# stanford-iprl-lab/nerf_shared

Hardware: AMD Instinct MI355X
Metric: rays_per_sec (higher is better)
Workload: dtype bf16; 1 GPU; lego_halfres_400x400_64c+128f_viewdirs_8x256_chunk4096; entry=Renderer.render(c2w=pose, retraw=False), chunk=4096, N_samples=64, N_importance=128, weights=random-init seeds 0/10, parallelism=single GPU

## Files before the change

nerf_shared_amd/csrc/capi.hip:

```cpp
#include <hip/hip_runtime.h>

#include <cmath>

#include <cstdio>
#include <cstring>
#include <mutex>
#include <utility>
#include <new>
#include <string>
#include <vector>

#include "kernels.h"
#include "program.h"

using namespace na;

namespace {
thread_local std::string g_err;

std::string lds_msg(const char *what, size_t bytes) {
    return std::string(what) + ": the per-ray scratch needs " + std::to_string(bytes) + " bytes of LDS per workgroup, the CU has " +
           std::to_string(LDS_LIMIT_BYTES) + " (fewer samples per ray)";
}

// ... 539 lines not shown
    if (Ni > 0 && !io->u && !io->t_lin_imp) return fail(NERF_AMD_EINVAL, "need u or t_lin_imp for sample_pdf");
    const nerf_amd_model *fm = fine ? fine : coarse;
    const int och = coarse->prog.out_ch;
    if (Ni > 0 && fm->prog.out_ch != och) return fail(NERF_AMD_EINVAL, "coarse and fine models disagree on output channels");
    if (och < 4) return fail(NERF_AMD_EINVAL, "field must output at least 4 channels");
    const bool has_vd = io->ray_ch > 8;
    if ((coarse->prog.arch.use_viewdirs != 0) != has_vd || (fm->prog.arch.use_viewdirs != 0) != has_vd)
        return fail(NERF_AMD_EINVAL, "ray batch width does not match the models' use_viewdirs");
    if (io->workspace_bytes < nerf_amd_render_rays_workspace(cfg, R, och) || !io->workspace)
        return fail(NERF_AMD_EINVAL, "workspace too small");
    p->cfg = cfg; p->coarse = coarse; p->fm = fm; p->io = io; p->R = R;
    p->Nc = Nc; p->Ni = Ni; p->Nf = Nf; p->och = och; p->has_vd = has_vd;

    char *w = static_cast<char *>(io->workspace);
    auto take = [&](size_t bytes) { float *q = reinterpret_cast<float *>(w); w += align_up(bytes); return q; };
    p->z_c = take(R * Nc * sizeof(float));
    p->raw_c = take(R * Nc * och * sizeof(float));
    p->w_c = take(R * Nc * sizeof(float));
    p->z_f = p->raw_f = nullptr;
    if (Ni > 0) {
        p->z_f = take(R * (size_t)Nf * sizeof(float));
        p->raw_f = take(R * (size_t)Nf * och * sizeof(float));
        if (io->z_vals) p->z_f = io->z_vals;
        if (io->raw) p->raw_f = io->raw;
    } else {
        if (io->z_vals) p->z_c = io->z_vals;
        if (io->raw) p->raw_c = io->raw;
        if (io->weights) p->w_c = io->weights;
    }
    return NERF_AMD_OK;
}

int stage_z(ChunkPlan &p, hipStream_t s) {
    const nerf_amd_render_io *io = p.io;
    int rc = 0;
    if (io->z_coarse) {
        if (p.Ni == 0 && io->z_vals)
            rc = hipMemcpyAsync(io->z_vals, io->z_coarse, p.R * p.Nc * sizeof(float), hipMemcpyDeviceToDevice, s) == hipSuccess
                     ? 0 : NERF_AMD_EHIP;
        else
            p.z_c = const_cast<float *>(io->z_coarse);
    } else {
        rc = launch_coarse_z(io->rays, io->ray_ch, io->t_vals, p.cfg->perturb ? io->t_rand : nullptr, p.R, p.Nc,
                             p.cfg->lindisp, p.cfg->perturb, p.z_c, s);
    }
    return rc ? fail(rc, "coarse_z launch failed") : NERF_AMD_OK;
}

int stage_field(const ChunkPlan &p, bool fine_pass, hipStream_t s) {
    MlpArgs a;
    std::memset(&a, 0, sizeof(a));
    a.rays = p.io->rays; a.ray_stride = p.io->ray_ch;
    a.viewdirs = p.has_vd ? p.io->rays + 8 : nullptr; a.vd_stride = p.io->ray_ch;
    if (!fine_pass) {
        a.z_vals = p.z_c; a.P = p.R * p.Nc; a.S = p.Nc; a.out = p.raw_c;
        return run_field(p.coarse, a, p.cfg->precision, s);
    }
    a.z_vals = p.z_f; a.P = p.R * (int64_t)p.Nf; a.S = p.Nf; a.out = p.raw_f;
    return run_field(p.fm, a, p.cfg->precision, s);
}

CompositeJob final_job(const ChunkPlan &p) {
    const nerf_amd_render_io *io = p.io;
    CompositeJob j;
    std::memset(&j, 0, sizeof(j));
    const bool two_pass = p.Ni > 0;
    j.raw = two_pass ? p.raw_f : p.raw_c; j.raw_ch = p.och; j.z = two_pass ? p.z_f : p.z_c;
    j.rays_d = io->rays + 3; j.rays_d_stride = io->ray_ch;
    j.noise = p.cfg->use_noise ? (two_pass ? io->noise1 : io->noise0) : nullptr;
    j.R = p.R; j.S = two_pass ? p.Nf : p.Nc; j.white_bkgd = p.cfg->white_bkgd;
    j.rgb = io->rgb_map; j.disp = io->disp_map; j.acc = io->acc_map; j.weights = two_pass ? io->weights : p.w_c;
    return j;
}

int stage_final(const ChunkPlan &p, hipStream_t s) {
    const CompositeJob j = final_job(p);
    int rc = launch_composite(j.raw, j.raw_ch, j.z, j.rays_d, j.rays_d_stride, j.noise, j.R, j.S, j.white_bkgd, j.rgb, j.disp,
                              j.acc, j.weights, nullptr, s);
    return rc ? fail(rc, "composite launch failed") : NERF_AMD_OK;
}

int stage_mid(const ChunkPlan &p, const ChunkPlan *prev, hipStream_t s) {
    const nerf_amd_render_io *io = p.io;
    CompositeJob cj;
    std::memset(&cj, 0, sizeof(cj));
    cj.raw = p.raw_c; cj.raw_ch = p.och; cj.z = p.z_c; cj.rays_d = io->rays + 3; cj.rays_d_stride = io->ray_ch;
    cj.noise = p.cfg->use_noise ? io->noise0 : nullptr; cj.R = p.R; cj.S = p.Nc; cj.white_bkgd = p.cfg->white_bkgd;
    cj.rgb = io->rgb0; cj.disp = io->disp0; cj.acc = io->acc0; cj.weights = nullptr;
    ResampleJob rj;
    std::memset(&rj, 0, sizeof(rj));
    rj.u = io->u; rj.t_lin = io->t_lin_imp; rj.Ni = p.Ni; rj.z_fine = p.z_f; rj.z_std = io->z_std;
    CompositeJob fj;
    if (prev) fj = final_job(*prev);
    int rc = launch_mid_stage(cj, rj, prev ? &fj : nullptr, s);
    if (rc == NERF_AMD_EINVAL && resample_lds_bytes(p.Nc, p.Ni, true) > LDS_LIMIT_BYTES)
        return fail(rc, lds_msg("render_rays (compositing + resampling)", resample_lds_bytes(p.Nc, p.Ni, true)));
    return rc ? fail(rc, "composite/resample launch failed") : NERF_AMD_OK;
}
}

extern "C" {

int nerf_amd_render_rays(const nerf_amd_render_cfg *cfg, const nerf_amd_model *coarse, const nerf_amd_model *fine,
                         const nerf_amd_render_io *io, int64_t R, void *stream) {
    if (R == 0 && cfg && coarse && io) return NERF_AMD_OK;
    ChunkPlan p;
    int rc = plan_chunk(cfg, coarse, fine, io, R, &p);
    if (rc) return rc;
    hipStream_t s = static_cast<hipStream_t>(stream);
    if ((rc = stage_z(p, s)) || (rc = stage_field(p, false, s))) return rc;
    if (p.Ni == 0) return stage_final(p, s);
    if ((rc = stage_mid(p, nullptr, s)) || (rc = stage_field(p, true, s))) return rc;
// ... 340 lines not shown
```

nerf_shared_amd/csrc/kernels.h:

```cpp
#pragma once
#include <hip/hip_runtime.h>
#include <stdint.h>
#include <atomic>
#include <vector>

#include "program.h"

namespace na {

struct MlpArgs {
    const uint16_t *stream_bf16;
    const float *bias_bf16;
    const uint16_t *stream_s16;
    const float *bias_s16;
    const uint16_t *stream_split;
    const float *stream_f32;
    const float *bias_f32;
    const LayerF32 *layers;
    int32_t n_layers;
    int32_t input_ch, input_ch_views, W, lds_rows;
    int32_t multires, multires_views, i_embed;
    const float *embedded;
    const float *pts;
    const float *rays;
    const float *z_vals;
    const float *viewdirs;
    int32_t ray_stride, vd_stride;
    int64_t P;
    int32_t S;
    int32_t out_ch;
    float *out;
    unsigned *tile_ctr;
    uint16_t *sv_e;
    uint16_t *sv_d;
    uint16_t *sv_h;
    uint16_t *sv_feat;
    uint16_t *sv_hv;
    uint8_t *sv_bits;
    const float *g_raw;
    uint16_t *g_rawb;
    uint16_t *g_rawt;
    uint16_t *g_hv;
    uint16_t *g_feat;
    uint16_t *g_h;
    const uint16_t *stream_bwd;
    float *g_pts;
    float *g_rays;
    float *g_vd;
    uint16_t *sv_e_lo, *sv_d_lo, *sv_h_lo, *sv_feat_lo, *sv_hv_lo;
    uint16_t *g_rawt_lo, *g_hv_lo, *g_feat_lo, *g_h_lo;
    const uint16_t *stream_bwd_split;
    float *g_scale;
#ifdef NERF_AMD_STAMPS
    unsigned long long *stamps;
#endif
};

constexpr int64_t pad_points(int64_t P) { return (P + 255) & ~(int64_t)255; }

unsigned *tile_counter_slot(int device);
unsigned *tile_counter_for(bool deal, hipStream_t s);
int tile_counters_init(int device);
extern std::atomic<int> g_variant;
bool mlp_bf16_supported(int multires, int multires_views, int use_viewdirs);
int launch_mlp_bf16(const MlpArgs &a, int multires, int multires_views, int use_viewdirs,
                    int n_frags_used, int n_tiles, hipStream_t s);
int launch_mlp_f32(const MlpArgs &a, hipStream_t s);
bool mlp_split_supported(int multires, int multires_views, int use_viewdirs, int out_ch);
int launch_mlp_split(const MlpArgs &a, int multires, int multires_views, int use_viewdirs, int n_frags_used, int n_tiles,
                     hipStream_t s);
int launch_mlp_split_save(const MlpArgs &a, int multires, int multires_views, int use_viewdirs, int n_frags_used, int n_tiles,
                          hipStream_t s);
int launch_mlp_bwd_split(const MlpArgs &a, int multires, int multires_views, int use_viewdirs, int n_frags_used, hipStream_t s);
int launch_embed(const float *x, int64_t n, int multires, float *out, hipStream_t s);

constexpr int MAX_TENSORS = 72;
struct PtrTable { const float *p[MAX_TENSORS]; };

int launch_pack(const Program &p, const FragDesc *d_frags, const TileDesc *d_tiles, const LayerF32 *d_layers,
                const TensorDesc *d_tensors, const PtrTable &d_weight_ptrs, const PtrTable &d_bias_ptrs,
                uint16_t *stream_bf16, float *bias_bf16, float *stream_f32, float *bias_f32,
                const FragDesc *d_frags16, const TileDesc *d_tiles16, uint16_t *stream_s16, float *bias_s16,
                const FragDesc *d_frags_bwd, uint16_t *stream_bwd, const FragDesc *d_frags_split, uint16_t *stream_split,
                const FragDesc *d_frags_bwd_split, uint16_t *stream_bwd_split, const TrainLayerF32 *d_tlayers, float *stream_f32_t, int copies, hipStream_t s);
void pack_bf16_host(const Program &p, int shape, const float *const *w, const float *const *b, uint16_t *stream, float *bias);
// ... 80 lines not shown
```

nerf_shared_amd/csrc/mlp_bf16_s16.hip:

```cpp
#include <hip/hip_runtime.h>
#include <utility>

#include "kernels.h"
#include "launch_util.h"
#include "pipeline.h"
#include "program.h"

#ifdef NERF_AMD_EXPERIMENTS
#include "../../tools/experiments/save_variants.inc"
#endif
#ifndef NA_EXPERIMENT_SAVE_FRAGS_HOOK
#define NA_EXPERIMENT_SAVE_FRAGS_HOOK
#endif

namespace na {

#ifdef NERF_AMD_STAMPS
unsigned long long *g_stamp_buf = nullptr;
#define STAMP(var) const unsigned long long var = __builtin_amdgcn_s_memtime()
#else
#define STAMP(var)
#endif

#define MFMA16(a_, b_, c_) __builtin_amdgcn_mfma_f32_16x16x32_bf16(a_, b_, c_, 0, 0, 0)

template <class C, int NR, int NM>
__device__ __forceinline__ void sched_step() {
    if constexpr ((C::OPT & 4) != 0) {
        __builtin_amdgcn_sched_group_barrier(0x100, NR, 0);
        __builtin_amdgcn_sched_group_barrier(0x008, NM, 0);
    }
}

struct NoHook {
    template <class P, class K> __device__ __forceinline__ void operator()(P, K) const {}
};

template <int F0, int T, int K1, int K2, int NB, int NFRAGS, class C, class P = std::integral_constant<int, 0>, class H = NoHook>
__device__ __forceinline__ void tile_pair(C &c, const bf16x8 *x1, const bf16x8 *x2, f32x4 (&acc)[2][2], P p_ = P{}, H &&hook = H{}) {
    {
        const f32x4 b0 = *reinterpret_cast<const f32x4 *>(c.bias_half + T * 16);
        const f32x4 b1 = *reinterpret_cast<const f32x4 *>(c.bias_half + (T + 1) * 16);
        acc[0][0] = b0; acc[0][1] = b0; acc[1][0] = b1; acc[1][1] = b1;
    }
    static_for<K1>([&](auto k_) {
        constexpr int k = k_, n = F0 + 2 * k;
        const bf16x8 w0 = take<n, NB, NFRAGS>(c);
        const bf16x8 w1 = take<n + 1, NB, NFRAGS>(c);
        acc[0][0] = MFMA16(w0, x1[2 * k], acc[0][0]);
        acc[0][1] = MFMA16(w0, x1[2 * k + 1], acc[0][1]);
        acc[1][0] = MFMA16(w1, x1[2 * k], acc[1][0]);
        acc[1][1] = MFMA16(w1, x1[2 * k + 1], acc[1][1]);
        sched_step<C, 2, 4>();
        hook(p_, std::integral_constant<int, k>{});
    });
    static_for<K2>([&](auto k_) {
        constexpr int k = k_, n = F0 + 2 * K1 + 2 * k;
        const bf16x8 w0 = take<n, NB, NFRAGS>(c);
        const bf16x8 w1 = take<n + 1, NB, NFRAGS>(c);
        acc[0][0] = MFMA16(w0, x2[2 * k], acc[0][0]);
        acc[0][1] = MFMA16(w0, x2[2 * k + 1], acc[0][1]);
        acc[1][0] = MFMA16(w1, x2[2 * k], acc[1][0]);
        acc[1][1] = MFMA16(w1, x2[2 * k + 1], acc[1][1]);
        sched_step<C, 2, 4>();
        hook(p_, std::integral_constant<int, K1 + k>{});
    });
}

template <int F0, int T, int K1, int NB, int NFRAGS, class C>
__device__ __forceinline__ void tile_single(C &c, const bf16x8 *x1, f32x4 (&acc)[2]) {
    const f32x4 b0 = *reinterpret_cast<const f32x4 *>(c.bias_half + T * 16);
    acc[0] = b0; acc[1] = b0;
    static_for<K1>([&](auto k_) {
        constexpr int k = k_, n = F0 + k;
        const bf16x8 w0 = take<n, NB, NFRAGS>(c);
        acc[0] = MFMA16(w0, x1[2 * k], acc[0]);
        acc[1] = MFMA16(w0, x1[2 * k + 1], acc[1]);
        sched_step<C, 1, 2>();
    });
}

typedef __attribute__((ext_vector_type(4))) unsigned u32x4;

template <bool RELU, bool PKRELU = true>
__device__ __forceinline__ bf16x8 pack_pair(const f32x4 &even, const f32x4 &odd) {
    bf16x8 y;
#pragma unroll
    for (int r = 0; r < 4; ++r) {
        float a = even[r], b = odd[r];
        if (RELU && !PKRELU) { a = relu_bits(a); b = relu_bits(b); }
        y[r] = (__bf16)a;
        y[4 + r] = (__bf16)b;
    }
    if (RELU && PKRELU) {
        u32x4 v = __builtin_bit_cast(u32x4, y);
#pragma unroll
        for (int i = 0; i < 4; ++i) {
            unsigned d = v[i];
            asm("v_pk_max_i16 %0, %1, 0" : "=v"(d) : "v"(d));
            v[i] = d;
        }
        y = __builtin_bit_cast(bf16x8, v);
    }
    return y;
}

template <int F0, int T0, int NPAIR, int K1, int K2, bool RELU, int NB, int NFRAGS, class C, class H = NoHook>
__device__ __forceinline__ void layer16(C &c, const bf16x8 *x1, const bf16x8 *x2, bf16x8 *y, H &&hook = H{}) {
    static_for<NPAIR>([&](auto p_) {
        constexpr int p = p_;
        f32x4 acc[2][2];
        tile_pair<F0 + p * 2 * (K1 + K2), T0 + 2 * p, K1, K2, NB, NFRAGS>(c, x1, x2, acc, p_, hook);
        y[2 * p] = pack_pair<RELU, !(C::OPT & 1)>(acc[0][0], acc[1][0]);
        y[2 * p + 1] = pack_pair<RELU, !(C::OPT & 1)>(acc[0][1], acc[1][1]);
    });
}

template <int L, int K>
struct Enc16 {
    static constexpr int NSTEP = (L + 1) / 2, CAP = 8 * K;
    static constexpr int N_EVEN = gen16_ntrig(L, 0), N_ODD = gen16_ntrig(L, 1);
    static constexpr int N_COMMON = N_ODD < N_EVEN ? N_ODD : N_EVEN;
    static constexpr int N_TAIL = (N_EVEN > N_ODD ? N_EVEN : N_ODD) - N_COMMON;
    float x[3], ra[3], tl[3], phase;
    unsigned sgn[3];
    float tail[N_TAIL > 0 ? N_TAIL : 1];

    __device__ __forceinline__ void begin(float x0, float x1, float x2, int h, int b) {
        constexpr float INV2PI_HI = 0.15915494f;
        constexpr float INV2PI_LO = (float)(0.15915494309189535 - (double)INV2PI_HI);
        x[0] = x0; x[1] = x1; x[2] = x2;
        phase = h ? 0.25f : 0.0f;
        const float s0 = b ? 2.0f : 1.0f;
#pragma unroll
// ... 33 lines not shown
    }
};

template <int L, int K, int STRIDE>
__device__ __forceinline__ void encode16(float x0, float x1, float x2, int h, int b, bf16x8 *out) {
    Enc16<L, K> e;
    e.begin(x0, x1, x2, h, b);
    static_for<Enc16<L, K>::NSTEP>([&](auto s_) { e.template step<s_, STRIDE>(out); });
    e.template finish<STRIDE>(h, b, out);
}

template <int NK, int ROW>
__device__ __forceinline__ void save_frags(uint16_t *base, const bf16x8 *y, const int64_t (&pidx)[2], int q) {
    NA_EXPERIMENT_SAVE_FRAGS_HOOK
    static_for<NK>([&](auto k_) {
        constexpr int k = k_;
        static_for<2>([&](auto cc_) {
            constexpr int cc = cc_;
            *reinterpret_cast<bf16x8 *>(base + pidx[cc] * ROW + k * 32 + q * 8) = y[2 * k + cc];
        });
    });
}

template <int NK>
__device__ __forceinline__ void save_bits(uint8_t *base, const bf16x8 *y, const int64_t (&pidx)[2], int q) {
    static_assert(NK == 4 || NK == 8, "one or two dwords of mask bits");
    static_for<2>([&](auto cc_) {
        constexpr int cc = cc_;
        unsigned w[NK / 4];
#pragma unroll
        for (int i = 0; i < NK / 4; ++i) w[i] = 0;
        static_for<NK>([&](auto k_) {
            constexpr int k = k_;
            const u32x4 v = __builtin_bit_cast(u32x4, y[2 * k + cc]);
            unsigned t = 0;
#pragma unroll
            for (int i = 0; i < 4; ++i) {
                unsigned m;
                asm("v_pk_min_u16 %0, %1, %2" : "=v"(m) : "v"(v[i]), "v"(0x00010001u));
                t |= m << i;
            }
            w[k / 4] |= t << (4 * (k % 4));
        });
        uint8_t *dst = base + pidx[cc] * (4 * NK) + q * NK;
        if constexpr (NK == 8) {
            typedef __attribute__((ext_vector_type(2))) unsigned u32x2;
            u32x2 o = {w[0], w[1]};
            *reinterpret_cast<u32x2 *>(dst) = o;
        } else {
            *reinterpret_cast<unsigned *>(dst) = w[0];
        }
    });
}

template <int LX, int LD, bool VD>
struct Layout16 {
    static constexpr int KE = gen16_ksteps(LX);
    static constexpr int KD = VD ? gen16_ksteps(LD) : 0;
    static constexpr int F_L0 = 0;
    static constexpr int F_L1 = F_L0 + 16 * KE;
    static constexpr int F_L5 = F_L1 + 4 * 128;
    static constexpr int F_L6 = F_L5 + 16 * (KE + 8);
    static constexpr int F_HEAD = F_L6 + 2 * 128;
    static constexpr int F_FEAT = F_HEAD;
    static constexpr int F_ALPHA = F_FEAT + 128;
    static constexpr int F_VIEWS = F_ALPHA + 8;
    static constexpr int F_RGB = F_VIEWS + 8 * (8 + KD);
    static constexpr int F_END = VD ? F_RGB + 4 : F_HEAD + 8;
    static constexpr int N_TILES = VD ? 128 + 16 + 1 + 8 + 1 : 128 + 1;
};

template <int LX, int LD, bool VD, class C, bool SAVE = false>
__global__ __launch_bounds__(C::WAVES * 64, 2) void mlp_bf16_s16_kernel(MlpArgs a) {
    constexpr int WG_THREADS = C::WAVES * 64, WG_POINTS = C::WAVES * 32;
    using Lay = Layout16<LX, LD, VD>;
    constexpr int KE = Lay::KE, KD = Lay::KD, NF = Lay::F_END, NB = (NF + C::BF - 1) / C::BF;
    extern __shared__ __attribute__((aligned(16))) char smem[];
    float *bias_lds = reinterpret_cast<float *>(smem + C::RING_BYTES);

    const int tid = threadIdx.x;
    const int lane = tid & 63;
    const int q = lane >> 4;
    C c;
    c.wave = __builtin_amdgcn_readfirstlane(tid >> 6);
    c.lag = __builtin_amdgcn_readfirstlane(c.wave >= C::WAVES / 2 ? 1 : 0);
    c.phase = __builtin_amdgcn_readfirstlane(C::N_PHASES == 4 ? ((c.wave + 2 * (c.wave >> 2)) & 3) : (c.wave >= C::WAVES / 2 ? 2 : 0));
    if constexpr ((C::OPT & 16) != 0) {
        if (c.lag) __builtin_amdgcn_s_setprio(1);
    }
    c.gstream = reinterpret_cast<const char *>(a.stream_s16) + lane * 16;
    c.ring_lane = smem + lane * 16;
    c.ring_u32 = (uint32_t)(uintptr_t)smem;
    c.bias_half = bias_lds + q * 4;
    if constexpr ((C::OPT & 64) != 0) {
        c.rsrc = make_rsrc(a.stream_s16, (unsigned)(NB * C::BLOCK_BYTES));
        c.rsrc_next = c.rsrc;
        c.lane16 = lane * 16;
        c.wave_off = c.wave * C::PIECES * 1024;
    }

    for (int i = tid; i < Lay::N_TILES * 16; i += WG_THREADS) bias_lds[i] = a.bias_s16[i];

    const int64_t n_point_tiles = (a.P + WG_POINTS - 1) / WG_POINTS;
    lds_u32_t *ticket_lds = (lds_u32_t *)(uintptr_t)(uint32_t)(uintptr_t)(bias_lds + Lay::N_TILES * 16);
    const bool dynamic = a.tile_ctr != nullptr;
#pragma unroll 1
// ... 108 lines not shown
                *reinterpret_cast<f32x4 *>(a.out + 4 * pidx[cc]) = o;
            }
        });
    } else {
        f32x4 o[2];
        tile_single<Lay::F_HEAD, 128, 8, NB, NF>(c, B, o);
        static_for<2>([&](auto cc_) {
            constexpr int cc = cc_;
            if (valid[cc]) {
#pragma unroll
                for (int r = 0; r < 4; ++r) {
                    const int row = 4 * q + r;
                    if (row < a.out_ch) a.out[(int64_t)a.out_ch * pidx[cc] + row] = o[cc][r];
                }
            }
        });
    }
    STAMP(t2);
    asm volatile("s_waitcnt vmcnt(0)" ::: "memory");
    if (dynamic && tid == 0) *ticket_lds = gridDim.x + ticket;
    __syncthreads();
    tile = dynamic ? (int64_t)*ticket_lds : tile + gridDim.x;
#ifdef NERF_AMD_STAMPS
    if (a.stamps && lane == 0) {
        const unsigned long long t3 = __builtin_amdgcn_s_memtime();
        unsigned long long *o = a.stamps + ((size_t)blockIdx.x * C::WAVES + c.wave) * 4;
        o[0] += t1 - t0; o[1] += t2 - t1; o[2] += t3 - t2; o[3] += 1;
    }
#endif
    }
    if (dynamic && tid == 0) {
        if (atomicAdd(a.tile_ctr + 1, 1u) == gridDim.x - 1) { a.tile_ctr[0] = 0u; a.tile_ctr[1] = 0u; }
    }
}


template <int LX, int LD, bool VD, class C>
__global__ __launch_bounds__(C::WAVES * 64, 2) void mlp_bf16_s16p_kernel(MlpArgs a) {
    static_assert((C::OPT & 32) != 0 && C::PHASE > 0, "the pipelined kernel needs the continuous ring");
    constexpr int WG_THREADS = C::WAVES * 64, WG_POINTS = C::WAVES * 32;
    using Lay = Layout16<LX, LD, VD>;
    constexpr int KE = Lay::KE, KD = Lay::KD, NF = Lay::F_END, NB = (NF + C::BF - 1) / C::BF;
    constexpr int SHIFT = NB % C::NS;
    using EncX = Enc16<LX, KE>;
    using EncD = Enc16<(VD ? LD : 1), (VD ? KD : 1)>;
    constexpr int NSX = EncX::NSTEP, NSD = VD ? EncD::NSTEP : 0;
    constexpr int PT_SLOTS = 4 + NSX + ((4 + NSX) & 1);
    constexpr int SLOT_LOAD = 1, SLOT_PTS = 3, SLOT_ENC = 4;
    static_assert(C::BF == 16 && C::PHASE == 8, "hook slots are laid out for a sync in front of k-step 4");
    static_assert(2 * PT_SLOTS <= 32 && 3 + 2 * NSD <= 16, "the encodings must fit on the hooks they are given");
    extern __shared__ __attribute__((aligned(16))) char smem[];
    float *bias_lds = reinterpret_cast<float *>(smem + C::RING_BYTES);
    lds_u32_t *ticket_lds = (lds_u32_t *)(uintptr_t)(uint32_t)(uintptr_t)(bias_lds + Lay::N_TILES * 16);

    const int tid = threadIdx.x;
    const int lane = tid & 63;
    const int q = lane >> 4;
    const int64_t n_point_tiles = (a.P + WG_POINTS - 1) / WG_POINTS;
    int64_t tile = blockIdx.x;
    if (tile >= n_point_tiles) return;
    int64_t tile_n = tile + gridDim.x;
    const bool dynamic = a.tile_ctr != nullptr;
    C c;
    c.wave = __builtin_amdgcn_readfirstlane(tid >> 6);
    c.lag = __builtin_amdgcn_readfirstlane(c.wave >= C::WAVES / 2 ? 1 : 0);
    c.phase = __builtin_amdgcn_readfirstlane(C::N_PHASES == 4 ? ((c.wave + 2 * (c.wave >> 2)) & 3) : (c.wave >= C::WAVES / 2 ? 2 : 0));
    c.gstream = reinterpret_cast<const char *>(a.stream_s16) + lane * 16;
    c.gstream_next = c.gstream;
    c.ring_lane = smem + lane * 16;
    c.ring_u32 = (uint32_t)(uintptr_t)smem;
#pragma unroll
    for (int i = 0; i < C::NS; ++i) {
        c.slot_u32[i] = c.ring_u32 + i * C::BLOCK_BYTES;
        c.slot_lane[i] = c.slot_u32[i] + lane * 16;
    }
    if constexpr ((C::OPT & 64) != 0) {
        c.rsrc = make_rsrc(a.stream_s16, (unsigned)(NB * C::BLOCK_BYTES));
        c.rsrc_next = c.rsrc;
        c.lane16 = lane * 16;
        c.wave_off = c.wave * C::PIECES * 1024;
    }
    c.bias_half = bias_lds + q * 4;
    for (int i = tid; i < Lay::N_TILES * 16; i += WG_THREADS) bias_lds[i] = a.bias_s16[i];

    float ld[7], dvn[2][3];
    float xsn[3];
    const int32_t P32 = (int32_t)a.P;
    const int32_t lane_pt = c.wave * 32 + (lane & 15);
    auto point_index = [&](int64_t t, int cc) { return (int32_t)t * WG_POINTS + lane_pt + cc * 16; };
    auto issue_loads = [&](int64_t t, int cc) {
        const int32_t p = point_index(t, cc);
        const int64_t pc = p < P32 ? p : P32 - 1;
        if (a.pts) {
            ld[0] = a.pts[3 * pc + 0]; ld[1] = a.pts[3 * pc + 1]; ld[2] = a.pts[3 * pc + 2];
        } else {
            const float *r = a.rays + (int64_t)((uint32_t)pc / (uint32_t)a.S) * a.ray_stride;
#pragma unroll
            for (int k = 0; k < 6; ++k) ld[k] = r[k];
            ld[6] = a.z_vals[pc];
        }
    };
    auto issue_dir_loads = [&]() {
        if constexpr (VD) {
#pragma unroll
            for (int cc = 0; cc < 2; ++cc) {
                const int32_t p = point_index(tile, cc);
                const int64_t pc = p < P32 ? p : P32 - 1;
                const float *d = a.viewdirs + (int64_t)((uint32_t)pc / (uint32_t)a.S) * a.vd_stride;
                dvn[cc][0] = d[0]; dvn[cc][1] = d[1]; dvn[cc][2] = d[2];
            }
        }
    };
    auto make_point = [&]() {
        if (a.pts) {
            xsn[0] = ld[0]; xsn[1] = ld[1]; xsn[2] = ld[2];
        } else {
            xsn[0] = mul_then_add(ld[3], ld[6], ld[0]);
            xsn[1] = mul_then_add(ld[4], ld[6], ld[1]);
            xsn[2] = mul_then_add(ld[5], ld[6], ld[2]);
        }
    };

    bf16x8 E[KE * 2];
    bf16x8 Dv[(VD ? KD : 1) * 2];
    static_for<2>([&](auto cc_) {
        constexpr int cc = cc_;
        issue_loads(tile, cc);
        make_point();
        encode16<LX, KE, 2>(xsn[0], xsn[1], xsn[2], q >> 1, q & 1, E + cc);
    });
    pipeline_prologue<NB>(c);
    asm volatile("s_waitcnt lgkmcnt(0)" ::: "memory");

    unsigned ticket = 0;
    const unsigned ticket_lds_addr = (unsigned)(uintptr_t)ticket_lds;
    const int tk_sel = __builtin_amdgcn_readfirstlane(dynamic ? c.wave : 1);
// ... 49 lines not shown
    auto hook_feat = [&](auto p_, auto k_) {
        constexpr int p = p_, k = k_;
        if constexpr (VD && (k == 0 || k == 4)) {
            constexpr int slot = 2 * p + (k == 4);
            if constexpr (slot == 1) issue_dir_loads();
            if constexpr (slot >= 3 && slot < 3 + 2 * NSD) {
                constexpr int cc = (slot - 3) / NSD, st = (slot - 3) % NSD;
                if constexpr (st == 0) ed.begin(dvn[cc][0], dvn[cc][1], dvn[cc][2], q >> 1, q & 1);
                ed.template step<st, 2>(Dv + cc);
                if constexpr (st == NSD - 1) ed.template finish<2>(q >> 1, q & 1, Dv + cc);
            }
        }
    };
    auto hook6 = [&](auto p_, auto k_) {
        constexpr int p = p_, k = k_;
        if constexpr (k == 0 || k == 4) prepare(std::integral_constant<int, 2 * p + (k == 4)>{});
    };
    auto hook7 = [&](auto p_, auto k_) {
        constexpr int p = p_, k = k_;
        if constexpr (k == 0 || k == 4) prepare(std::integral_constant<int, 16 + 2 * p + (k == 4)>{});
    };

#ifdef NERF_AMD_STAMPS
    unsigned long long t_prev = __builtin_amdgcn_s_memtime();
#endif
#pragma unroll 1
    for (;;) {
#ifdef NERF_AMD_STAMPS
    if (a.stamps && lane == 0) {
        const unsigned long long t_now = __builtin_amdgcn_s_memtime();
        unsigned long long *o = a.stamps + ((size_t)blockIdx.x * C::WAVES + c.wave) * 4;
        o[1] += t_now - t_prev; o[3] += 1;
        t_prev = t_now;
    }
#endif
    c.has_next = tile_n < n_point_tiles;
    asm volatile("" : "+v"(c.gstream));
    c.gstream_next = c.gstream;

    block_sync<-1, NB>(c);
    static_for<C::LA>([&](auto i_) { constexpr int i = i_; c.q[i] = ring_frag<i>(c); });

    bf16x8 A[16], B[16];
    layer16<Lay::F_L0, 0, 8, KE, 0, true, NB, NF>(c, E, E, A);
    layer16<Lay::F_L1 + 0 * 128, 16, 8, 8, 0, true, NB, NF>(c, A, A, B);
    layer16<Lay::F_L1 + 1 * 128, 32, 8, 8, 0, true, NB, NF>(c, B, B, A);
    layer16<Lay::F_L1 + 2 * 128, 48, 8, 8, 0, true, NB, NF>(c, A, A, B);
    layer16<Lay::F_L1 + 3 * 128, 64, 8, 8, 0, true, NB, NF>(c, B, B, A);
    layer16<Lay::F_L5, 80, 8, KE, 8, true, NB, NF>(c, E, A, B);
    layer16<Lay::F_L6, 96, 8, 8, 0, true, NB, NF>(c, B, B, A, hook6);
    layer16<Lay::F_L6 + 128, 112, 8, 8, 0, true, NB, NF>(c, A, A, B, hook7);

    if constexpr (VD) {
        layer16<Lay::F_FEAT, 128, 8, 8, 0, false, NB, NF>(c, B, B, A, hook_feat);
        f32x4 alpha[2], rgb[2];
        tile_single<Lay::F_ALPHA, 144, 8, NB, NF>(c, B, alpha);
        layer16<Lay::F_VIEWS, 145, 4, 8, KD, true, NB, NF>(c, A, Dv, B);
        tile_single<Lay::F_RGB, 153, 4, NB, NF>(c, B, rgb);
        static_for<2>([&](auto cc_) {
            constexpr int cc = cc_;
            const int32_t p = point_index(tile, cc);
            if (p < P32 && q == 0) {
                f32x4 o = {rgb[cc][0], rgb[cc][1], rgb[cc][2], alpha[cc][0]};
                *reinterpret_cast<f32x4 *>(a.out + 4 * (int64_t)p) = o;
            }
        });
    } else {
        f32x4 o[2];
        tile_single<Lay::F_HEAD, 128, 8, NB, NF>(c, B, o);
        static_for<2>([&](auto cc_) {
            constexpr int cc = cc_;
            const int32_t p = point_index(tile, cc);
            if (p < P32) {
#pragma unroll
                for (int r = 0; r < 4; ++r) {
                    const int row = 4 * q + r;
                    if (row < a.out_ch) a.out[(int64_t)a.out_ch * p + row] = o[cc][r];
                }
            }
        });
    }
    if (!c.has_next) break;
    tile = tile_n;
    tile_n = dynamic ? (int64_t)*ticket_lds : tile + gridDim.x;
    if constexpr (SHIFT != 0) {
        uint32_t sl[C::NS], su[C::NS];
#pragma unroll
        for (int i = 0; i < C::NS; ++i) { sl[i] = c.slot_lane[(i + SHIFT) % C::NS]; su[i] = c.slot_u32[(i + SHIFT) % C::NS]; }
#pragma unroll
        for (int i = 0; i < C::NS; ++i) { c.slot_lane[i] = sl[i]; c.slot_u32[i] = su[i]; }
    }
    }
#ifdef NERF_AMD_STAMPS
    if (a.stamps && lane == 0) {
        unsigned long long *o = a.stamps + ((size_t)blockIdx.x * C::WAVES + c.wave) * 4;
        unsigned xcc;
        asm volatile("s_getreg_b32 %0, hwreg(HW_REG_XCC_ID)" : "=s"(xcc));
        o[0] = wall_clock64();
        o[2] = xcc & 15;
    }
#endif
    asm volatile("s_waitcnt vmcnt(0)" ::: "memory");
    if (dynamic && tid == 0) {
        if (atomicAdd(a.tile_ctr + 1, 1u) == gridDim.x - 1) { a.tile_ctr[0] = 0u; a.tile_ctr[1] = 0u; }
    }
}

namespace {
constexpr int TILE_CTR_SLOTS = 1024;
unsigned *g_tile_ctr[16] = {};
std::atomic<unsigned> g_tile_ctr_next{0};
}

int tile_counters_init(int device) {
    if (device < 0 || device >= 16) return NERF_AMD_EINVAL;
    if (g_tile_ctr[device]) return NERF_AMD_OK;
    unsigned *p = nullptr;
    if (hipMalloc(reinterpret_cast<void **>(&p), TILE_CTR_SLOTS * 2 * sizeof(unsigned)) != hipSuccess) return NERF_AMD_EHIP;
    if (hipMemset(p, 0, TILE_CTR_SLOTS * 2 * sizeof(unsigned)) != hipSuccess) { (void)hipFree(p); return NERF_AMD_EHIP; }
    g_tile_ctr[device] = p;
    return NERF_AMD_OK;
}

unsigned *tile_counter_slot(int device) {
    if (device < 0 || device >= 16 || !g_tile_ctr[device]) return nullptr;
    return g_tile_ctr[device] + 2 * (g_tile_ctr_next.fetch_add(1, std::memory_order_relaxed) % TILE_CTR_SLOTS);
}

unsigned *tile_counter_for(bool deal, hipStream_t s) {
    if (!deal) return nullptr;
    hipStreamCaptureStatus st = hipStreamCaptureStatusNone;
    if (hipStreamIsCapturing(s, &st) != hipSuccess || st != hipStreamCaptureStatusNone) return nullptr;
    int dev = 0;
    return hipGetDevice(&dev) == hipSuccess ? tile_counter_slot(dev) : nullptr;
}

template <int LX, int LD, bool VD, class C>
static int launch_wg16p(const MlpArgs &a, int n_frags_used, int n_tiles, hipStream_t s) {
    constexpr int WG_THREADS = C::WAVES * 64, WG_POINTS = C::WAVES * 32;
    using Lay = Layout16<LX, LD, VD>;
    if (n_frags_used != Lay::F_END || n_tiles != Lay::N_TILES) return NERF_AMD_EINVAL;
    const size_t lds = C::RING_BYTES + (size_t)Lay::N_TILES * 16 * sizeof(float) + 16;
    static DynamicLdsOptIn opt_in;
    if (opt_in.ensure(reinterpret_cast<const void *>(mlp_bf16_s16p_kernel<LX, LD, VD, C>), lds) != hipSuccess) return NERF_AMD_EHIP;
    int64_t groups = (a.P + WG_POINTS - 1) / WG_POINTS;
    if (groups <= 0) return NERF_AMD_OK;
    if (a.P >= (int64_t)1 << 31) return NERF_AMD_EINVAL;
    const int n_cu = device_cu_count();
    const bool deal = groups > 2 * (int64_t)n_cu && g_variant != 42;
    if (groups > n_cu) groups = n_cu;
    MlpArgs a2 = a;
    a2.tile_ctr = tile_counter_for(deal, s);
#ifdef NERF_AMD_STAMPS
    a2.stamps = g_stamp_buf;
#endif
    hipLaunchKernelGGL((mlp_bf16_s16p_kernel<LX, LD, VD, C>), dim3((unsigned)groups), dim3(WG_THREADS), lds, s, a2);
    return hipGetLastError() == hipSuccess ? NERF_AMD_OK : NERF_AMD_EHIP;
}

template <int LX, int LD, bool VD, class C, bool SAVE = false>
static int launch_wg16(const MlpArgs &a, int n_frags_used, int n_tiles, hipStream_t s) {
    constexpr int WG_THREADS = C::WAVES * 64, WG_POINTS = C::WAVES * 32;
    using Lay = Layout16<LX, LD, VD>;
    if (n_frags_used != Lay::F_END || n_tiles != Lay::N_TILES) return NERF_AMD_EINVAL;
    const size_t lds = C::RING_BYTES + (size_t)Lay::N_TILES * 16 * sizeof(float) + 16;
    static DynamicLdsOptIn opt_in;
    if (opt_in.ensure(reinterpret_cast<const void *>(mlp_bf16_s16_kernel<LX, LD, VD, C, SAVE>), lds) != hipSuccess)
        return NERF_AMD_EHIP;
    int64_t groups = (a.P + WG_POINTS - 1) / WG_POINTS;
    if (groups <= 0) return NERF_AMD_OK;
    if (a.P >= (int64_t)1 << 31) return NERF_AMD_EINVAL;
    bool deal = false;
    if (g_variant != 31) {
        const int n_wg = device_cu_count() * (8 / C::WAVES);
        deal = groups > 2 * (int64_t)n_wg && g_variant != 42;
        if (groups > n_wg) groups = n_wg;
    }
    MlpArgs a2 = a;
    a2.tile_ctr = tile_counter_for(deal, s);
#ifdef NERF_AMD_STAMPS
    a2.stamps = g_stamp_buf;
#endif
    hipLaunchKernelGGL((mlp_bf16_s16_kernel<LX, LD, VD, C, SAVE>), dim3((unsigned)groups), dim3(WG_THREADS), lds, s, a2);
    return hipGetLastError() == hipSuccess ? NERF_AMD_OK : NERF_AMD_EHIP;
}

using Cfg16 = Ctx<8, 16, 4, 8, 4, 0, 1, 4 + 8 + 64>;
using Cfg16R1 = Ctx<8, 16, 4, 8, 2>;
using Cfg16P = Ctx<8, 16, 4, 8, 4, 0, 1, 4 + 8 + 32 + 64>;
#ifndef NA_EXPERIMENT_SAVE_CFG
template <int LX, int LD> using CfgSaveT = Ctx<8, 16, 4, 8, 2>;
#endif

#ifdef NERF_AMD_EXPERIMENTS
#include "../../tools/experiments/field_variants_s16.inc"
#endif

int launch_mlp_bf16_s16(const MlpArgs &a, int multires, int multires_views, int use_viewdirs,
                        int n_frags_used, int n_tiles, hipStream_t s) {
#ifdef NERF_AMD_EXPERIMENTS
    {
        int rc_x = NERF_AMD_EUNSUPPORTED;
        if (experiment_launch_s16(a, multires, multires_views, use_viewdirs, n_frags_used, n_tiles, s, &rc_x)) return rc_x;
    }
#endif
// ... 40 lines not shown
```

nerf_shared_amd/csrc/pipeline.h:

```cpp
#pragma once
#include <hip/hip_runtime.h>
#include <utility>

namespace na {

typedef __attribute__((ext_vector_type(8))) __bf16 bf16x8;
typedef __attribute__((ext_vector_type(16))) float f32x16;
typedef __attribute__((ext_vector_type(4))) float f32x4;

template <int N, class F, int... Is>
__device__ __forceinline__ void static_for_impl(F &&f, std::integer_sequence<int, Is...>) {
    (f(std::integral_constant<int, Is>{}), ...);
}
template <int N, class F>
__device__ __forceinline__ void static_for(F &&f) {
    static_for_impl<N>(f, std::make_integer_sequence<int, N>{});
}

struct NoLedger {
    static constexpr int stores_before(int) { return 0; }
};
template <int WAVES_, int BF_, int NS_, int PHASE_, int LA_ = 0, int ABL_ = 0, int NP_ = 1, int OPT_ = 0, class LEDGER_ = NoLedger>
struct Ctx {
    using Ledger = LEDGER_;
    static constexpr int WAVES = WAVES_, BF = BF_, NS = NS_, PHASE = PHASE_, LA = LA_, ABL = ABL_, NP = NP_, OPT = OPT_;
    static constexpr int WAVES_PER_SIMD = (WAVES_ * NP_ >= 8 && NP_ == 1) ? 2 : 1;
    static_assert(LA_ == 0 || (PHASE_ > 0 && LA_ <= PHASE_ && PHASE_ + LA_ <= BF_), "read-ahead would cross an unpublished block");
    bf16x8 q[LA_ > 0 ? LA_ : 1];
    static constexpr int PIECES = BF / WAVES;
    static constexpr int BLOCK_BYTES = BF * 1024;
    static constexpr int RING_BYTES = NS * BLOCK_BYTES;
    static constexpr int LOOKAHEAD = PHASE > 0 ? 1 : 0;
    static constexpr int N_PHASES = (OPT_ & 128) ? 4 : (OPT_ & 8) ? 2 : 1;
    static_assert(BF % WAVES == 0 && NS >= 3 && PHASE < BF, "bad pipeline shape");
    const char *gstream;
    const char *ring_lane;
    uint32_t ring_u32;
    const float *bias_half;
    int wave;
    int lag;
    int phase;
    uint32_t slot_lane[NS_];
    uint32_t slot_u32[NS_];
    const char *gstream_next;
    int has_next;
    typedef __attribute__((ext_vector_type(4))) unsigned rsrc_t;
    rsrc_t rsrc, rsrc_next;
    unsigned lane16;
    unsigned wave_off;
};

__device__ __forceinline__ __attribute__((ext_vector_type(4))) unsigned make_rsrc(const void *base, unsigned bytes) {
    const unsigned long long b = (unsigned long long)(uintptr_t)base;
    __attribute__((ext_vector_type(4))) unsigned r;
// ... 117 lines not shown

template <int n, int NB, int NFRAGS, class C>
__device__ __forceinline__ void late_issue(const C &c) {
    if constexpr (C::N_PHASES > 1 && C::PHASE > 0) {
        static_for<3>([&](auto i_) {
            constexpr int ph = i_ + 1;
            if constexpr (C::N_PHASES == 4 || ph == 2) {
                constexpr int off = C::PHASE + ph * (C::BF / 4);
                if constexpr ((n - off) % C::BF == 0 && n - off >= -C::BF) {
                    constexpr int B = (n - off) / C::BF;
                    if constexpr (B >= -1 && B + C::LOOKAHEAD < NB) sync_issue<B, NB, ph>(c);
                }
                if constexpr (n == 0 && off < C::BF && -1 + C::LOOKAHEAD < NB) sync_issue<-1, NB, ph>(c);
                if constexpr (n == NFRAGS - 1) {
                    static_for<2>([&](auto j_) {
                        constexpr int B = NB - 2 - j_;
                        if constexpr (B >= 0 && B * C::BF + off > NFRAGS - 1) sync_issue<B, NB, ph>(c);
                    });
                }
            }
        });
    }
}

template <int NB, class C>
__device__ __forceinline__ void pipeline_prologue(const C &c) {
    if constexpr (C::ABL & 1) return;
    static_for<C::NS - 1 - C::LOOKAHEAD>([&](auto b_) { constexpr int b = b_; if constexpr (b < NB) issue_block<b>(c); });
}

template <int n, class C>
__device__ __forceinline__ bf16x8 ring_frag(const C &c) {
    if constexpr ((C::OPT & 32) != 0)
        return *(lds_frag_t *)(uintptr_t)(c.slot_lane[(n / C::BF) % C::NS] + ((n % C::BF) << 10));
    else
        return *reinterpret_cast<const bf16x8 *>(c.ring_lane + ((n % (C::NS * C::BF)) << 10));
}

template <int n, int NB, class C>
__device__ __forceinline__ void maybe_sync(const C &c) {
    if constexpr ((C::OPT & 2) != 0) {
        static_assert(C::PHASE == C::BF / 2 && C::LA <= C::PHASE, "stagger is written for a mid-block sync");
        if constexpr (n % C::BF == C::PHASE && (n / C::BF + 1) < NB) {
            if (!c.lag) block_sync<n / C::BF, NB>(c);
        }
        if constexpr (n % C::BF == 0 && (n / C::BF + 1) < NB) {
            if (c.lag) block_sync<n / C::BF, NB>(c);
        }
    } else {
        if constexpr (n % C::BF == C::PHASE && (n / C::BF + C::LOOKAHEAD) < NB) block_sync<n / C::BF, NB>(c);
    }
}

template <int n, int NB, int NFRAGS, class C>
__device__ __forceinline__ bf16x8 take(C &c) {
    maybe_sync<n, NB>(c);
    late_issue<n, NB, NFRAGS>(c);
    if constexpr (C::ABL & 2) {
        bf16x8 f = c.q[0];
        asm volatile("" : "+v"(f));
        return f;
    } else if constexpr (C::LA == 0) {
        return ring_frag<n>(c);
    } else {
        const bf16x8 f = c.q[n % C::LA];
        if constexpr (n + C::LA < NFRAGS) c.q[n % C::LA] = ring_frag<n + C::LA>(c);
        return f;
    }
}

template <int F0, int N, int NB, int NFRAGS, class C>
__device__ __forceinline__ void skip_frags(C &c) {
    static_for<N>([&](auto i_) {
        constexpr int n = F0 + i_;
        maybe_sync<n, NB>(c);
        late_issue<n, NB, NFRAGS>(c);
        if constexpr (C::LA > 0 && (C::ABL & 2) == 0) {
            if constexpr (n + C::LA >= F0 + N && n + C::LA < NFRAGS) c.q[n % C::LA] = ring_frag<n + C::LA>(c);
        }
    });
}

__device__ __forceinline__ float mul_then_add(float a, float b, float c) {
    float m = a * b;
    asm volatile("" : "+v"(m));
    return m + c;
}

__device__ __forceinline__ float relu_bits(float v) {
    int i = __builtin_bit_cast(int, v);
    return __builtin_bit_cast(float, i > 0 ? i : 0);
}

}
```

Before: 4.866 million rays/s.

## Skip feature and view-direction layers for wavefronts whose points all have zero density

The alpha head is now computed first from weights kept resident in LDS, read straight from the weight stream, so density is known before the feature, view and RGB layers run. If skip_empty is set (output is not the returned raw and noise is off) and no point in the wavefront has positive alpha, the kernel only advances the fragment pipeline through the remaining stages and writes zero RGB. Zero-density samples add no colour, so the composited result stays the same. The read-ahead queue is reworked to step over the hole left by the alpha fragments. In exchange the kernel needs 8 KB more LDS, which may lower occupancy, and the work is skipped only when every point in a wavefront is empty.

```diff
diff --git a/nerf_shared_amd/csrc/capi.hip b/nerf_shared_amd/csrc/capi.hip
--- a/nerf_shared_amd/csrc/capi.hip
+++ b/nerf_shared_amd/csrc/capi.hip
@@ -615,12 +615,10 @@
     std::memset(&a, 0, sizeof(a));
     a.rays = p.io->rays; a.ray_stride = p.io->ray_ch;
     a.viewdirs = p.has_vd ? p.io->rays + 8 : nullptr; a.vd_stride = p.io->ray_ch;
-    if (!fine_pass) {
-        a.z_vals = p.z_c; a.P = p.R * p.Nc; a.S = p.Nc; a.out = p.raw_c;
-        return run_field(p.coarse, a, p.cfg->precision, s);
-    }
-    a.z_vals = p.z_f; a.P = p.R * (int64_t)p.Nf; a.S = p.Nf; a.out = p.raw_f;
-    return run_field(p.fm, a, p.cfg->precision, s);
+    if (!fine_pass) { a.z_vals = p.z_c; a.P = p.R * p.Nc; a.S = p.Nc; a.out = p.raw_c; }
+    else { a.z_vals = p.z_f; a.P = p.R * (int64_t)p.Nf; a.S = p.Nf; a.out = p.raw_f; }
+    a.skip_empty = (a.out != p.io->raw && !p.cfg->use_noise) ? 1 : 0;
+    return run_field(fine_pass ? p.fm : p.coarse, a, p.cfg->precision, s);
 }
 
 CompositeJob final_job(const ChunkPlan &p) {
diff --git a/nerf_shared_amd/csrc/kernels.h b/nerf_shared_amd/csrc/kernels.h
--- a/nerf_shared_amd/csrc/kernels.h
+++ b/nerf_shared_amd/csrc/kernels.h
@@ -31,6 +31,7 @@
     int32_t out_ch;
     float *out;
     unsigned *tile_ctr;
+    int32_t skip_empty;
     uint16_t *sv_e;
     uint16_t *sv_d;
     uint16_t *sv_h;
diff --git a/nerf_shared_amd/csrc/mlp_bf16_s16.hip b/nerf_shared_amd/csrc/mlp_bf16_s16.hip
--- a/nerf_shared_amd/csrc/mlp_bf16_s16.hip
+++ b/nerf_shared_amd/csrc/mlp_bf16_s16.hip
@@ -8,9 +8,14 @@
 
 #ifdef NERF_AMD_EXPERIMENTS
 #include "../../tools/experiments/save_variants.inc"
+#include "../../tools/experiments/skip_variants.inc"
 #endif
 #ifndef NA_EXPERIMENT_SAVE_FRAGS_HOOK
 #define NA_EXPERIMENT_SAVE_FRAGS_HOOK
+#endif
+#ifndef NA_EXPERIMENT_ALWAYS_DRY
+#define NA_EXPERIMENT_ALWAYS_DRY(flag) false
+#define NA_EXPERIMENT_SKIP_VARIANT(args)
 #endif
 
 namespace na {
@@ -80,6 +85,23 @@
     });
 }
 
+template <int T, int NK, class C>
+__device__ __forceinline__ void tile_single_resident(const C &c, uint32_t frag_lane, const bf16x8 *x1, f32x4 (&acc)[2]) {
+    const f32x4 b0 = *reinterpret_cast<const f32x4 *>(c.bias_half + T * 16);
+    acc[0] = b0; acc[1] = b0;
+    bf16x8 w[NK];
+    static_for<NK>([&](auto k_) { constexpr int k = k_; w[k] = *(lds_frag_t *)(uintptr_t)(frag_lane + (k << 10)); });
+    static_for<NK>([&](auto k_) {
+        constexpr int k = k_;
+        acc[0] = MFMA16(w[k], x1[2 * k], acc[0]);
+        acc[1] = MFMA16(w[k], x1[2 * k + 1], acc[1]);
+    });
+    if constexpr ((C::OPT & 4) != 0) {
+        __builtin_amdgcn_sched_group_barrier(0x100, NK, 0);
+        __builtin_amdgcn_sched_group_barrier(0x008, 2 * NK, 0);
+    }
+}
+
 typedef __attribute__((ext_vector_type(4))) unsigned u32x4;
 
 template <bool RELU, bool PKRELU = true>
@@ -219,6 +241,9 @@
         }
     });
 }
+
+template <class C, int F0, int N>
+struct WithHole : C { static constexpr int HOLE0 = F0, HOLEN = N; };
 
 template <int LX, int LD, bool VD>
 struct Layout16 {
@@ -433,6 +458,8 @@
     extern __shared__ __attribute__((aligned(16))) char smem[];
     float *bias_lds = reinterpret_cast<float *>(smem + C::RING_BYTES);
     lds_u32_t *ticket_lds = (lds_u32_t *)(uintptr_t)(uint32_t)(uintptr_t)(bias_lds + Lay::N_TILES * 16);
+    char *alpha_lds = reinterpret_cast<char *>(bias_lds + Lay::N_TILES * 16) + 16;
+    static_assert((C::RING_BYTES + Lay::N_TILES * 64 + 16) % 16 == 0, "resident fragments are read 16 bytes per lane");
 
     const int tid = threadIdx.x;
     const int lane = tid & 63;
@@ -442,7 +469,7 @@
     if (tile >= n_point_tiles) return;
     int64_t tile_n = tile + gridDim.x;
     const bool dynamic = a.tile_ctr != nullptr;
-    C c;
+    WithHole<C, (VD ? Lay::F_ALPHA : -1), (VD ? 8 : 0)> c;
     c.wave = __builtin_amdgcn_readfirstlane(tid >> 6);
     c.lag = __builtin_amdgcn_readfirstlane(c.wave >= C::WAVES / 2 ? 1 : 0);
     c.phase = __builtin_amdgcn_readfirstlane(C::N_PHASES == 4 ? ((c.wave + 2 * (c.wave >> 2)) & 3) : (c.wave >= C::WAVES / 2 ? 2 : 0));
@@ -463,6 +490,12 @@
     }
     c.bias_half = bias_lds + q * 4;
     for (int i = tid; i < Lay::N_TILES * 16; i += WG_THREADS) bias_lds[i] = a.bias_s16[i];
+    if constexpr (VD) {
+        static_assert(WG_THREADS * 16 == 8 * 1024, "one 16-byte piece per thread");
+        reinterpret_cast<u32x4 *>(alpha_lds)[tid] = reinterpret_cast<const u32x4 *>(a.stream_s16 + (size_t)Lay::F_ALPHA * 512)[tid];
+    }
+    const uint32_t alpha_lane = (uint32_t)(uintptr_t)alpha_lds + lane * 16;
+    const int skip_empty = __builtin_amdgcn_readfirstlane(a.skip_empty);
 
     float ld[7], dvn[2][3];
     float xsn[3];
@@ -618,11 +651,23 @@
     layer16<Lay::F_L6 + 128, 112, 8, 8, 0, true, NB, NF>(c, A, A, B, hook7);
 
     if constexpr (VD) {
-        layer16<Lay::F_FEAT, 128, 8, 8, 0, false, NB, NF>(c, B, B, A, hook_feat);
         f32x4 alpha[2], rgb[2];
-        tile_single<Lay::F_ALPHA, 144, 8, NB, NF>(c, B, alpha);
-        layer16<Lay::F_VIEWS, 145, 4, 8, KD, true, NB, NF>(c, A, Dv, B);
-        tile_single<Lay::F_RGB, 153, 4, NB, NF>(c, B, rgb);
+        tile_single_resident<144, 8>(c, alpha_lane, B, alpha);
+        bool live = false;
+        static_for<2>([&](auto cc_) {
+            constexpr int cc = cc_;
+            live = live || (point_index(tile, cc) < P32 && !(alpha[cc][0] <= 0.0f));
+        });
+        const bool dry = skip_empty != 0 && (NA_EXPERIMENT_ALWAYS_DRY(skip_empty) || __builtin_amdgcn_ballot_w64(live && q == 0) == 0);
+        if (dry) {
+            pass_frags<Lay::F_FEAT, NF - Lay::F_FEAT, NB, NF>(c);
+            rgb[0] = f32x4{0.0f, 0.0f, 0.0f, 0.0f}; rgb[1] = rgb[0];
+        } else {
+            layer16<Lay::F_FEAT, 128, 8, 8, 0, false, NB, NF>(c, B, B, A, hook_feat);
+            pass_frags<Lay::F_ALPHA, 8, NB, NF>(c);
+            layer16<Lay::F_VIEWS, 145, 4, 8, KD, true, NB, NF>(c, A, Dv, B);
+            tile_single<Lay::F_RGB, 153, 4, NB, NF>(c, B, rgb);
+        }
         static_for<2>([&](auto cc_) {
             constexpr int cc = cc_;
             const int32_t p = point_index(tile, cc);
@@ -706,7 +751,7 @@
     constexpr int WG_THREADS = C::WAVES * 64, WG_POINTS = C::WAVES * 32;
     using Lay = Layout16<LX, LD, VD>;
     if (n_frags_used != Lay::F_END || n_tiles != Lay::N_TILES) return NERF_AMD_EINVAL;
-    const size_t lds = C::RING_BYTES + (size_t)Lay::N_TILES * 16 * sizeof(float) + 16;
+    const size_t lds = C::RING_BYTES + (size_t)Lay::N_TILES * 16 * sizeof(float) + 16 + (VD ? 8 * 1024 : 0);
     static DynamicLdsOptIn opt_in;
     if (opt_in.ensure(reinterpret_cast<const void *>(mlp_bf16_s16p_kernel<LX, LD, VD, C>), lds) != hipSuccess) return NERF_AMD_EHIP;
     int64_t groups = (a.P + WG_POINTS - 1) / WG_POINTS;
@@ -717,6 +762,9 @@
     if (groups > n_cu) groups = n_cu;
     MlpArgs a2 = a;
     a2.tile_ctr = tile_counter_for(deal, s);
+    if (g_variant == 64) a2.skip_empty = 0;
+    else if (g_variant == 65) a2.skip_empty = 1;
+    NA_EXPERIMENT_SKIP_VARIANT(a2)
 #ifdef NERF_AMD_STAMPS
     a2.stamps = g_stamp_buf;
 #endif
diff --git a/nerf_shared_amd/csrc/pipeline.h b/nerf_shared_amd/csrc/pipeline.h
--- a/nerf_shared_amd/csrc/pipeline.h
+++ b/nerf_shared_amd/csrc/pipeline.h
@@ -1,5 +1,6 @@
 #pragma once
 #include <hip/hip_runtime.h>
+#include <type_traits>
 #include <utility>
 
 namespace na {
@@ -223,8 +224,15 @@
     }
 }
 
+template <class C, class = void>
+struct Hole { static constexpr int F0 = -1, N = 0; };
+template <class C>
+struct Hole<C, std::void_t<decltype(C::HOLE0)>> { static constexpr int F0 = C::HOLE0, N = C::HOLEN; };
+
 template <int n, int NB, int NFRAGS, class C>
 __device__ __forceinline__ bf16x8 take(C &c) {
+    using H = Hole<C>;
+    static_assert(n < H::F0 || n >= H::F0 + H::N, "a fragment of the hole is passed (pass_frags), never taken");
     maybe_sync<n, NB>(c);
     late_issue<n, NB, NFRAGS>(c);
     if constexpr (C::ABL & 2) {
@@ -234,10 +242,23 @@
     } else if constexpr (C::LA == 0) {
         return ring_frag<n>(c);
     } else {
-        const bf16x8 f = c.q[n % C::LA];
-        if constexpr (n + C::LA < NFRAGS) c.q[n % C::LA] = ring_frag<n + C::LA>(c);
+        constexpr bool has_hole = H::N > 0;
+        constexpr int m = (has_hole && n >= H::F0 + H::N) ? n - H::N : n;
+        constexpr int r = (has_hole && m + C::LA >= H::F0) ? m + C::LA + H::N : m + C::LA;
+        static_assert(!has_hole || (H::F0 % C::BF == 0 && H::N + C::LA <= C::BF), "read-ahead over the hole would cross an unpublished block");
+        const bf16x8 f = c.q[m % C::LA];
+        if constexpr (r < NFRAGS) c.q[m % C::LA] = ring_frag<r>(c);
         return f;
     }
+}
+
+template <int F0, int N, int NB, int NFRAGS, class C>
+__device__ __forceinline__ void pass_frags(C &c) {
+    static_for<N>([&](auto i_) {
+        constexpr int n = F0 + i_;
+        maybe_sync<n, NB>(c);
+        late_issue<n, NB, NFRAGS>(c);
+    });
 }
 
 template <int F0, int N, int NB, int NFRAGS, class C>
```

Measured after the change: 5.454 million rays/s (median of 6 runs). +12.1%, better.
